# dluvizon/deephar

Measured on NVIDIA H100. Metric: frames/sec (256x256, 16-frame clips, b32), higher is better.
Workload: dtype bf16x3 split (fp32 accumulate, wgmma)

## Files before the change

deephar_b200/csrc/conv_patch.cu:

```cuda
#include "tc_common.cuh"

namespace tcd {
using namespace tc;
using R = tc::Roles<2>;
constexpr int WARP_EPI0 = R::WARP_EPI0, WARP_TMA = R::WARP_TMA, WARP_PATCH = R::WARP_PATCH, NTHREADS = R::NTHREADS,
              REGS_PROD = R::REGS_PROD, REGS_EPI = R::REGS_EPI, REGS_CTRL = R::REGS_CTRL;

constexpr int NWG = 128;
constexpr int NA = 4;
constexpr int NB = 3;
constexpr int MAX_NP = 8;

template <bool LO>
__global__ void __launch_bounds__(NTHREADS, 1)
patch_dense_kernel(const __grid_constant__ PatchParams PP, const __grid_constant__ CUtensorMap map_hi,
                   const __grid_constant__ CUtensorMap map_lo, const __grid_constant__ CUtensorMap map_x) {
    const TcParams& P = PP.t;
    extern __shared__ __align__(1024) uint8_t smem_raw[];
    if (smem_u32(smem_raw) & 1023u) __trap();
    uint8_t* smem = smem_raw;
    const int tid = threadIdx.x;
    const int warp = tid >> 5, lane = tid & 31;
    constexpr bool want_lo = LO;
    const int b_bytes = P.bn_cta * 64;
    uint8_t* b_ring = smem + NA * 2 * A_BYTES;
    uint8_t* patch0 = b_ring + NB * 2 * b_bytes;
    uint64_t* bars = reinterpret_cast<uint64_t*>(patch0 + (size_t)PP.np * PP.patch_stride);
    float* post = reinterpret_cast<float*>(bars + 64);
    constexpr int NB_A = NA + 2 * NA;
    constexpr int NB_P = NB_A + 2 * NB;
    const uint32_t bar_full0 = smem_u32(bars), bar_empty0 = smem_u32(bars + NA), bar_fullb0 = smem_u32(bars + NB_A),
                   bar_emptyb0 = smem_u32(bars + NB_A + NB), bar_pfull0 = smem_u32(bars + NB_P),
                   bar_pempty0 = smem_u32(bars + NB_P + MAX_NP);
    const int n0 = blockIdx.y * P.bn_cta;
    const int nkb = P.n_kblocks;
    const int ntaps = PP.ntaps, ncb = PP.ncb, np = PP.np;

    if (warp == WARP_TMA && lane == 0) {
        tma_prefetch_desc(&map_hi);
        if (want_lo) tma_prefetch_desc(&map_lo);
        tma_prefetch_desc(&map_x);
        for (int s = 0; s < NA; ++s) {
            mbar_init(bar_full0 + 8 * s, (uint32_t)NWG);
            mbar_init(bar_empty0 + 16 * s, 1u);
            mbar_init(bar_empty0 + 16 * s + 8, 1u);
        }
        for (int s = 0; s < NB; ++s) {
            mbar_init(bar_fullb0 + 8 * s, 1);
            mbar_init(bar_emptyb0 + 8 * s, 1);
        }
        for (int s = 0; s < MAX_NP; ++s) {
            mbar_init(bar_pfull0 + 8 * s, 1);
            mbar_init(bar_pempty0 + 8 * s, ntaps == 1 ? (uint32_t)NWG : (uint32_t)(2 * NWG));
        }
        fence_barrier_init();
    }
    __syncthreads();

    const int tiles_mine = ((int)P.n_mtiles - (int)blockIdx.x + (int)gridDim.x - 1) / (int)gridDim.x;
    const int total_g = tiles_mine * nkb;
    const int n_patches = tiles_mine * ncb;
    const int rows_per_tile = BM / PP.tw;

    if (warp < WARP_EPI0) {
        reg_prod<REGS_PROD, R::LAUNCH_REGS>();
        const ConvParams& c = P.c;
        const int w = warp >> 2;
        const int tw = tid & (NWG - 1);
        const int ch4 = tw & 7;
        const int prow = tw >> 3;
        uint32_t poff[8];
        int yy[8], xx[8];
#pragma unroll
        for (int i = 0; i < 8; ++i) {
            const int m = prow + 16 * i;
            const int ty = m / PP.tw, tx = m - ty * PP.tw;
            const int f = ty / PP.ry, r = ty - f * PP.ry;
            poff[i] = (uint32_t)(((f * PP.pr + r * PP.sh) * PP.pc + tx * PP.sw) * (SBK * 4) + ch4 * 16);
            yy[i] = r * PP.sh - PP.pt;
            xx[i] = tx * PP.sw - PP.pl;
        }
        const uint32_t patch_s = smem_u32(patch0);
        const bool relu = c.pre_relu != 0, has_bn = c.pre_scale != nullptr;
        uint32_t aoff[8];
#pragma unroll
        for (int i = 0; i < 8; ++i) aoff[i] = swz64(prow + 16 * i, ch4 * 4);
        int tap = w % ntaps, p = w / ntaps;
        int cb = p % ncb, ti = p / ncb;
        int slot = p % np;
        uint32_t pphase = (uint32_t)(p / np) & 1u;
        int ky = tap / PP.kw, kx = tap - ky * PP.kw;
        int s = w % NA;
        uint32_t it = 0;
        int cb_loaded = -1, ti_masked = -1;
        float4 ps = make_float4(1.f, 1.f, 1.f, 1.f), pb = make_float4(0.f, 0.f, 0.f, 0.f);
        int y0 = 0;
        for (int g = w; g < total_g; g += 2) {
            if (has_bn && cb != cb_loaded) {
                cb_loaded = cb;
                const int ci = cb * SBK + ch4 * 4;
                if (ci < c.Cin) {
                    ps = __ldg(reinterpret_cast<const float4*>(c.pre_scale + ci));
                    pb = __ldg(reinterpret_cast<const float4*>(c.pre_shift + ci));
                } else {
                    ps = make_float4(0.f, 0.f, 0.f, 0.f);
                    pb = make_float4(0.f, 0.f, 0.f, 0.f);
                }
            }
            unsigned okmask = 0xffu;
            if (PP.mask) {
                if (ti != ti_masked) {
                    ti_masked = ti;
                    const int t = blockIdx.x + ti * gridDim.x;
                    y0 = PP.fn > 1 ? 0 : (t * rows_per_tile) % PP.rows_per_frame;
                }
                okmask = 0;
#pragma unroll
                for (int i = 0; i < 8; ++i) {
                    const int iy = y0 * PP.sh + yy[i] + ky, ix = xx[i] + kx;
                    if ((unsigned)iy < (unsigned)PP.vh && (unsigned)ix < (unsigned)PP.vw) okmask |= 1u << i;
                }
            }
            mbar_wait(bar_pfull0 + 8 * slot, pphase);
            const uint32_t base = patch_s + (uint32_t)slot * (uint32_t)PP.patch_stride +
                                  (uint32_t)((ky * PP.pc + kx) * (SBK * 4));
            float4 v[8];
#pragma unroll
            for (int i = 0; i < 8; ++i) v[i] = lds128(base + poff[i]);

            wait_stage_free(bar_empty0, s, it);
            const uint32_t a_hi = smem_u32(smem) + (uint32_t)s * (2 * A_BYTES);
            const uint32_t a_lo = a_hi + A_BYTES;
#pragma unroll
            for (int i = 0; i < 8; ++i) {
                float4 t4 = v[i];
                if (has_bn) {
                    t4.x = fmaf(t4.x, ps.x, pb.x); t4.y = fmaf(t4.y, ps.y, pb.y);
                    t4.z = fmaf(t4.z, ps.z, pb.z); t4.w = fmaf(t4.w, ps.w, pb.w);
                }
                if (relu) {
                    t4.x = fmaxf(t4.x, 0.f); t4.y = fmaxf(t4.y, 0.f); t4.z = fmaxf(t4.z, 0.f); t4.w = fmaxf(t4.w, 0.f);
                }
                if (!((okmask >> i) & 1u)) t4 = make_float4(0.f, 0.f, 0.f, 0.f);
                uint32_t h0, l0, h1, l1;
                split2(t4.x, t4.y, h0, l0);
                split2(t4.z, t4.w, h1, l1);
                asm volatile("st.shared.v2.b32 [%0], {%1, %2};" ::"r"(a_hi + aoff[i]), "r"(h0), "r"(h1) : "memory");
                if (want_lo) asm volatile("st.shared.v2.b32 [%0], {%1, %2};" ::"r"(a_lo + aoff[i]), "r"(l0), "r"(l1) : "memory");
            }
            const bool last_of_patch = tap + 2 >= ntaps;
            if (last_of_patch) mbar_arrive(bar_pempty0 + 8 * slot);
            fence_proxy_async();
            mbar_arrive(bar_full0 + 8 * s);
            s += 2;
            if (s >= NA) { s -= NA; ++it; }
            tap += 2;
            kx += 2;
            while (tap >= ntaps) {
                tap -= ntaps;
                ++p;
                if (++cb == ncb) { cb = 0; ++ti; }
                if (++slot == np) { slot = 0; pphase ^= 1u; }
                ky = 0; kx = tap;
                if (kx >= PP.kw) { kx -= PP.kw; ky = 1; }
            }
            while (kx >= PP.kw) { kx -= PP.kw; ++ky; }
        }
    } else if (warp < WARP_TMA) {
        reg_inc<REGS_EPI>();
        stage_post<R::NEPI>(P, n0, post, tid - 32 * WARP_EPI0);
        const int wg = (warp - WARP_EPI0) >> 2, wt = tid - 32 * WARP_EPI0 - 128 * wg;
        pp_consumer<false, LO, NA, NB>(P, wg, wt, n0, tiles_mine, make_desc64(smem_u32(smem)), make_desc64(smem_u32(b_ring)),
                                       bar_full0, bar_empty0, bar_fullb0, bar_emptyb0, 0u, post, 0);
    } else {
        reg_dec<REGS_CTRL>();
        if (warp == WARP_TMA) {
            if (lane == 0) {
                const uint32_t tx = (uint32_t)(want_lo ? 2 : 1) * (uint32_t)b_bytes;
                for (int g = 0; g < total_g; ++g) {
                    const int p = g / ntaps, tap = g - p * ntaps;
                    const int cb = p % ncb;
                    const int kc = tap * P.c.Cin + cb * SBK;
                    const int sb = g % NB;
                    const uint32_t itb = (uint32_t)(g / NB);
                    if (itb >= 1) mbar_wait_relaxed(bar_emptyb0 + 8 * sb, (itb - 1) & 1, 0u);
                    const uint32_t full = bar_fullb0 + 8 * sb;
                    mbar_arrive_expect_tx(full, tx);
                    const uint32_t b_hi = smem_u32(b_ring + (size_t)sb * (2 * b_bytes));
                    const uint32_t b_lo = b_hi + (uint32_t)b_bytes;
                    tma_load_2d(b_hi, &map_hi, kc, n0, full);
                    if (want_lo) tma_load_2d(b_lo, &map_lo, kc, n0, full);
                }
            }
        } else if (warp == WARP_PATCH) {
            if (lane == 0) {
                for (int p = 0; p < n_patches; ++p) {
                    const int ti = p / ncb, cb = p - ti * ncb;
                    const int t = blockIdx.x + ti * gridDim.x;
                    const int grow = t * rows_per_tile;
                    const int nf = grow / PP.rows_per_frame;
                    const int y0 = grow - nf * PP.rows_per_frame;
                    const int slot = p % np;
                    const uint32_t u = (uint32_t)(p / np);
                    mbar_wait_relaxed(bar_pempty0 + 8 * slot, (u & 1u) ^ 1u, 0u);
                    const uint32_t pf = bar_pfull0 + 8 * slot;
                    mbar_arrive_expect_tx(pf, (uint32_t)PP.patch_bytes);
                    tma_load_4d(smem_u32(patch0 + (size_t)slot * PP.patch_stride), &map_x, cb * SBK, -PP.pl,
                                y0 * PP.sh - PP.pt, nf, pf);
                }
            }
        }
    }
}

static bool plan_geom(const ConvParams& p, PatchParams* g) {
    if (p.sh != 1 || p.sw != 1) return false;
    if (p.kh == 1 && p.kw == 1) {
        const int64_t hw = (int64_t)p.H * p.W;
        int vw = 128;
        while (vw > 1 && (hw % vw) != 0) vw >>= 1;
        if (vw < 8) return false;
        g->tw = vw; g->ry = tc::BM / vw; g->fn = 1; g->pc = vw; g->pr = g->ry;
        g->vw = vw; g->vh = (int)(((int64_t)p.N * hw) / vw);
        g->rows_per_frame = g->vh; g->pt = g->pl = 0; g->kw = 1; g->ntaps = 1;
        return true;
    }
    if (p.Ho != p.H || p.Wo != p.W) return false;
    if (!(p.W == 128 || p.W == 64 || p.W == 32 || p.W == 16 || p.W == 8)) return false;
    const int tr = tc::BM / p.W;
    if (tr <= p.H ? (p.H % tr) != 0 : (tr % p.H) != 0) return false;
    g->tw = p.W;
    g->ry = tr <= p.H ? tr : p.H;
    g->fn = tr <= p.H ? 1 : tr / p.H;
    g->pc = p.W + p.kw - 1;
    g->pr = g->ry + p.kh - 1;
    g->rows_per_frame = p.H; g->vh = p.H; g->vw = p.W;
    g->pt = p.pt; g->pl = p.pl; g->kw = p.kw; g->ntaps = p.kh * p.kw;
    return true;
}

}

bool dh_plan_patch(const dh_ctx* ctx, const ConvParams& p, const dh_packed_w* packed, int precision, tc::PatchPlan* pl) {
    using namespace tc;
    using namespace tcd;
    if (!ctx->dense_patch || !packed->lo) return false;
    if (p.M < 1) return false;
    if ((p.Cin & 7) || (p.ldx & 3) || (reinterpret_cast<uintptr_t>(p.x) & 15) || !bn_pro_aligned(p)) return false;
    if (!packed_fits(packed, p.kh * p.kw * p.Cin, p.Cout)) return false;
    PatchParams& PP = pl->k;
    if (!plan_geom(p, &PP)) return false;
    if (PP.pc > 256 || PP.pr > 256 || PP.fn > 256) return false;
    if ((int64_t)PP.vh * PP.vw * p.ldx * 4 >= (1ll << 40)) return false;
    TcParams& P = PP.t;
    P.c = p;
    P.c.K = p.kh * p.kw * p.Cin;
    P.k_pad = packed->k;
    PP.ncb = (p.Cin + SBK - 1) / SBK;
    P.n_kblocks = PP.ncb * PP.ntaps;
    int gy;
    tile_n(p.Cout, &P.bn_cta, &gy);
    P.precision = (precision == 1) ? 1 : 3;
    P.ks = 0;
    P.n_mtiles = (p.M + BM - 1) / BM;
    P.stages = 2;
    P.dbg = 0;
    PP.sh = 1; PP.sw = 1;
    PP.mask = (p.pre_scale != nullptr && PP.ntaps > 1) ? 1 : 0;
    PP.patch_bytes = SBK * 4 * PP.pc * PP.pr * PP.fn;
    PP.patch_stride = (PP.patch_bytes + 1023) / 1024 * 1024;
    const size_t fixed = (size_t)NA * 2 * A_BYTES + (size_t)NB * 2 * P.bn_cta * 64 + 512 + POST_SMEM;
    const int np = (int)((SMEM_LIMIT - fixed) / (size_t)PP.patch_stride);
    if (np < 2) return false;
    PP.np = np > MAX_NP ? MAX_NP : np;
    pl->w = packed;
    pl->gy = gy;
    pl->smem = fixed + (size_t)PP.np * PP.patch_stride;
    pl->cluster = false;
    return true;
}

int dh_launch_patch(const dh_ctx* ctx, const tc::PatchPlan& pl, cudaStream_t s) {
    using namespace tc;
    using namespace tcd;
    const PatchParams& PP = pl.k;
    const ConvParams& c = PP.t.c;
    const dh_packed_w* w = pl.w;
    const int vn = PP.ntaps == 1 ? 1 : c.N;
    CUtensorMap map_hi, map_lo, map_x;
    if (!make_map_w(&map_hi, w->hi, w->k, w->cout_pad, SBK, PP.t.bn_cta) ||
        !make_map_w(&map_lo, w->lo, w->k, w->cout_pad, SBK, PP.t.bn_cta) ||
        !make_map_x(&map_x, c.x, c.ldx, c.Cin, PP.vw, PP.vh, vn, PP.pc, PP.pr, PP.fn)) {
        dh_set_error("dh_launch_patch: cuTensorMapEncodeTiled failed");
        return -1;
    }
    return pick<true, false>(PP.t.precision == 3, [&](auto lo) {
        return launch_persistent<patch_dense_kernel<lo()>>("dh_launch_patch", ctx, pl, PP.t.n_mtiles, NTHREADS, s,
                                                           map_hi, map_lo, map_x);
    });
}
```

deephar_b200/csrc/tc_common.cuh:

```cuda
#pragma once
#include <cuda.h>
#include <cuda_bf16.h>
#include <type_traits>
#include "common.cuh"
#include "conv_params.cuh"

namespace tc {


constexpr int BM = 128;
constexpr int BK = 64;
constexpr int NPROD = 256;
constexpr int MAX_BN_CTA = 96;
constexpr int ACC_N = MAX_BN_CTA / 2;
constexpr int MH = BM / 64;
constexpr int BM64 = 64;
constexpr int MAX_BN_CTA64 = 144;
constexpr int bn_max(int bm) { return bm == BM64 ? MAX_BN_CTA64 : MAX_BN_CTA; }
template <int Q, int NPW = 2>
struct Roles {
    static constexpr int EPQ = Q;
    static constexpr int NEPI = 128 * Q;
    static constexpr int WARP_EPI0 = 4 * NPW;
    static constexpr int WARP_TMA = WARP_EPI0 + 4 * Q, WARP_PATCH = WARP_TMA + 2;
    static constexpr int NTHREADS = 32 * (WARP_TMA + 4);
    static constexpr int REGS_PROD = Q == 1 ? 168 : (NPW == 1 ? 192 : 88);
    static constexpr int REGS_EPI = Q == 2 && NPW == 2 ? 136 : 144, REGS_CTRL = 32;
    static constexpr int LAUNCH_REGS = NTHREADS <= 512 ? 128 : 96;
    static_assert(128 * NPW * REGS_PROD + NEPI * REGS_EPI + 128 * REGS_CTRL <= NTHREADS * LAUNCH_REGS,
                  "setmaxnreg budget exceeds the CTA's register allocation: the last setmaxnreg.inc would never return");
};
constexpr int A_TILE_BYTES = BM * 128;
constexpr int MAX_STAGES = 4;

struct TcParams {
    ConvParams c;
    int n_kblocks;
    int bn_cta;
    int stages;
    int precision;
    int ks;
    int k_pad;
    int n_mtiles;
    int dbg;
};

struct SepParams {
    TcParams t;
    int patch_stride;
    int patch_bytes;
    int ry, fn;
    int bm;
    int epi_smem;
    int dbg;
};

struct PatchParams {
    TcParams t;
    int np, patch_stride, patch_bytes;
    int ntaps, ncb;
    int tw;
    int ry, fn;
    int pc, pr;
    int rows_per_frame;
    int kw;
    int pt, pl, sh, sw;
    int vh, vw;
    int mask;
};

__device__ __forceinline__ void mbar_wait_relaxed(uint32_t bar, uint32_t parity, uint32_t ns) {
    uint32_t ok;
    for (;;) {
        asm volatile(
            "{\n .reg .pred p;\n mbarrier.try_wait.parity.shared::cta.b64 p, [%1], %2;\n selp.u32 %0, 1, 0, p;\n}"
            : "=r"(ok)
            : "r"(bar), "r"(parity)
            : "memory");
        if (ok) break;
        if (ns) __nanosleep(ns);
    }
}
__device__ __forceinline__ void fence_proxy_async() { asm volatile("fence.proxy.async.shared::cta;" ::: "memory"); }

__device__ __forceinline__ void tma_load_2d(uint32_t dst, const CUtensorMap* map, int c0, int c1, uint32_t bar) {
    asm volatile(
        "cp.async.bulk.tensor.2d.shared::cluster.global.mbarrier::complete_tx::bytes [%0], [%1, {%2, %3}], [%4];"
        ::"r"(dst), "l"(map), "r"(c0), "r"(c1), "r"(bar)
        : "memory");
}
__device__ __forceinline__ void tma_prefetch_desc(const CUtensorMap* map) {
    asm volatile("prefetch.tensormap [%0];" ::"l"(map) : "memory");
}
__device__ __forceinline__ void tma_store_2d(const CUtensorMap* map, uint32_t src, int c0, int c1) {
    asm volatile("cp.async.bulk.tensor.2d.global.shared::cta.bulk_group [%0, {%2, %3}], [%1];"
                 ::"l"(map), "r"(src), "r"(c0), "r"(c1)
                 : "memory");
}
__device__ __forceinline__ void bulk_commit() { asm volatile("cp.async.bulk.commit_group;" ::: "memory"); }
__device__ __forceinline__ void bulk_wait_read() { asm volatile("cp.async.bulk.wait_group.read 0;" ::: "memory"); }
__device__ __forceinline__ void bulk_s2peer(uint32_t dst_cluster, uint32_t src_cta, uint32_t bytes, uint32_t bar_cluster) {
    asm volatile("cp.async.bulk.shared::cluster.shared::cta.mbarrier::complete_tx::bytes [%0], [%1], %2, [%3];"
                 ::"r"(dst_cluster), "r"(src_cta), "r"(bytes), "r"(bar_cluster)
                 : "memory");
}
template <int R> __device__ __forceinline__ void reg_inc() { asm volatile("setmaxnreg.inc.sync.aligned.u32 %0;" ::"n"(R)); }
template <int R> __device__ __forceinline__ void reg_dec() { asm volatile("setmaxnreg.dec.sync.aligned.u32 %0;" ::"n"(R)); }
template <int R, int LAUNCH> __device__ __forceinline__ void reg_prod() {
    if constexpr (R > LAUNCH) reg_inc<R>();
    else if constexpr (R < LAUNCH) reg_dec<R>();
}
__device__ __forceinline__ void mbar_arrive_cluster(uint32_t bar_cluster) {
    asm volatile("mbarrier.arrive.release.cluster.shared::cluster.b64 _, [%0];" ::"r"(bar_cluster) : "memory");
}

__device__ __forceinline__ void wgmma_fence() { asm volatile("wgmma.fence.sync.aligned;" ::: "memory"); }
__device__ __forceinline__ void wgmma_commit() { asm volatile("wgmma.commit_group.sync.aligned;" ::: "memory"); }
template <int N> __device__ __forceinline__ void wgmma_wait() { asm volatile("wgmma.wait_group.sync.aligned %0;" ::"n"(N) : "memory"); }
__device__ __forceinline__ void acc_fence(float& r) { asm volatile("" : "+f"(r)::"memory"); }
template <int N> __device__ __forceinline__ void wgmma_bf16(float* d, uint64_t a, uint64_t b, uint32_t acc);
template <> __device__ __forceinline__ void wgmma_bf16<16>(float* d, uint64_t a, uint64_t b, uint32_t acc) {
    asm volatile(
        "{\n .reg .pred p;\n setp.ne.b32 p, %10, 0;\n"
        " wgmma.mma_async.sync.aligned.m64n16k16.f32.bf16.bf16 {%0, %1, %2, %3, %4, %5, %6, %7}, %8, %9, p, 1, 1, 0, 0;\n}"
        : "+f"(d[0]), "+f"(d[1]), "+f"(d[2]), "+f"(d[3]), "+f"(d[4]), "+f"(d[5]), "+f"(d[6]), "+f"(d[7])
        : "l"(a), "l"(b), "r"(acc));
}
template <> __device__ __forceinline__ void wgmma_bf16<32>(float* d, uint64_t a, uint64_t b, uint32_t acc) {
    asm volatile(
        "{\n .reg .pred p;\n setp.ne.b32 p, %18, 0;\n"
        " wgmma.mma_async.sync.aligned.m64n32k16.f32.bf16.bf16 {%0, %1, %2, %3, %4, %5, %6, %7, %8, %9, %10, %11, %12, %13, %14, %15}, %16, %17, p, 1, 1, 0, 0;\n}"
        : "+f"(d[0]), "+f"(d[1]), "+f"(d[2]), "+f"(d[3]), "+f"(d[4]), "+f"(d[5]), "+f"(d[6]), "+f"(d[7]), "+f"(d[8]), "+f"(d[9]), "+f"(d[10]), "+f"(d[11]), "+f"(d[12]), "+f"(d[13]), "+f"(d[14]), "+f"(d[15])
        : "l"(a), "l"(b), "r"(acc));
}
template <> __device__ __forceinline__ void wgmma_bf16<48>(float* d, uint64_t a, uint64_t b, uint32_t acc) {
    asm volatile(
        "{\n .reg .pred p;\n setp.ne.b32 p, %26, 0;\n"
        " wgmma.mma_async.sync.aligned.m64n48k16.f32.bf16.bf16 {%0, %1, %2, %3, %4, %5, %6, %7, %8, %9, %10, %11, %12, %13, %14, %15, %16, %17, %18, %19, %20, %21, %22, %23}, %24, %25, p, 1, 1, 0, 0;\n}"
        : "+f"(d[0]), "+f"(d[1]), "+f"(d[2]), "+f"(d[3]), "+f"(d[4]), "+f"(d[5]), "+f"(d[6]), "+f"(d[7]), "+f"(d[8]), "+f"(d[9]), "+f"(d[10]), "+f"(d[11]), "+f"(d[12]), "+f"(d[13]), "+f"(d[14]), "+f"(d[15]), "+f"(d[16]), "+f"(d[17]), "+f"(d[18]), "+f"(d[19]), "+f"(d[20]), "+f"(d[21]), "+f"(d[22]), "+f"(d[23])
        : "l"(a), "l"(b), "r"(acc));
}
template <> __device__ __forceinline__ void wgmma_bf16<64>(float* d, uint64_t a, uint64_t b, uint32_t acc) {
    asm volatile(
        "{\n .reg .pred p;\n setp.ne.b32 p, %34, 0;\n"
        " wgmma.mma_async.sync.aligned.m64n64k16.f32.bf16.bf16 {%0, %1, %2, %3, %4, %5, %6, %7, %8, %9, %10, %11, %12, %13, %14, %15, %16, %17, %18, %19, %20, %21, %22, %23, %24, %25, %26, %27, %28, %29, %30, %31}, %32, %33, p, 1, 1, 0, 0;\n}"
        : "+f"(d[0]), "+f"(d[1]), "+f"(d[2]), "+f"(d[3]), "+f"(d[4]), "+f"(d[5]), "+f"(d[6]), "+f"(d[7]), "+f"(d[8]), "+f"(d[9]), "+f"(d[10]), "+f"(d[11]), "+f"(d[12]), "+f"(d[13]), "+f"(d[14]), "+f"(d[15]), "+f"(d[16]), "+f"(d[17]), "+f"(d[18]), "+f"(d[19]), "+f"(d[20]), "+f"(d[21]), "+f"(d[22]), "+f"(d[23]), "+f"(d[24]), "+f"(d[25]), "+f"(d[26]), "+f"(d[27]), "+f"(d[28]), "+f"(d[29]), "+f"(d[30]), "+f"(d[31])
        : "l"(a), "l"(b), "r"(acc));
}
template <> __device__ __forceinline__ void wgmma_bf16<80>(float* d, uint64_t a, uint64_t b, uint32_t acc) {
    asm volatile(
        "{\n .reg .pred p;\n setp.ne.b32 p, %42, 0;\n"
        " wgmma.mma_async.sync.aligned.m64n80k16.f32.bf16.bf16 {%0, %1, %2, %3, %4, %5, %6, %7, %8, %9, %10, %11, %12, %13, %14, %15, %16, %17, %18, %19, %20, %21, %22, %23, %24, %25, %26, %27, %28, %29, %30, %31, %32, %33, %34, %35, %36, %37, %38, %39}, %40, %41, p, 1, 1, 0, 0;\n}"
        : "+f"(d[0]), "+f"(d[1]), "+f"(d[2]), "+f"(d[3]), "+f"(d[4]), "+f"(d[5]), "+f"(d[6]), "+f"(d[7]), "+f"(d[8]), "+f"(d[9]), "+f"(d[10]), "+f"(d[11]), "+f"(d[12]), "+f"(d[13]), "+f"(d[14]), "+f"(d[15]), "+f"(d[16]), "+f"(d[17]), "+f"(d[18]), "+f"(d[19]), "+f"(d[20]), "+f"(d[21]), "+f"(d[22]), "+f"(d[23]), "+f"(d[24]), "+f"(d[25]), "+f"(d[26]), "+f"(d[27]), "+f"(d[28]), "+f"(d[29]), "+f"(d[30]), "+f"(d[31]), "+f"(d[32]), "+f"(d[33]), "+f"(d[34]), "+f"(d[35]), "+f"(d[36]), "+f"(d[37]), "+f"(d[38]), "+f"(d[39])
        : "l"(a), "l"(b), "r"(acc));
}
template <> __device__ __forceinline__ void wgmma_bf16<96>(float* d, uint64_t a, uint64_t b, uint32_t acc) {
    asm volatile(
        "{\n .reg .pred p;\n setp.ne.b32 p, %50, 0;\n"
        " wgmma.mma_async.sync.aligned.m64n96k16.f32.bf16.bf16 {%0, %1, %2, %3, %4, %5, %6, %7, %8, %9, %10, %11, %12, %13, %14, %15, %16, %17, %18, %19, %20, %21, %22, %23, %24, %25, %26, %27, %28, %29, %30, %31, %32, %33, %34, %35, %36, %37, %38, %39, %40, %41, %42, %43, %44, %45, %46, %47}, %48, %49, p, 1, 1, 0, 0;\n}"
        : "+f"(d[0]), "+f"(d[1]), "+f"(d[2]), "+f"(d[3]), "+f"(d[4]), "+f"(d[5]), "+f"(d[6]), "+f"(d[7]), "+f"(d[8]), "+f"(d[9]), "+f"(d[10]), "+f"(d[11]), "+f"(d[12]), "+f"(d[13]), "+f"(d[14]), "+f"(d[15]), "+f"(d[16]), "+f"(d[17]), "+f"(d[18]), "+f"(d[19]), "+f"(d[20]), "+f"(d[21]), "+f"(d[22]), "+f"(d[23]), "+f"(d[24]), "+f"(d[25]), "+f"(d[26]), "+f"(d[27]), "+f"(d[28]), "+f"(d[29]), "+f"(d[30]), "+f"(d[31]), "+f"(d[32]), "+f"(d[33]), "+f"(d[34]), "+f"(d[35]), "+f"(d[36]), "+f"(d[37]), "+f"(d[38]), "+f"(d[39]), "+f"(d[40]), "+f"(d[41]), "+f"(d[42]), "+f"(d[43]), "+f"(d[44]), "+f"(d[45]), "+f"(d[46]), "+f"(d[47])
        : "l"(a), "l"(b), "r"(acc));
}

template <> __device__ __forceinline__ void wgmma_bf16<144>(float* d, uint64_t a, uint64_t b, uint32_t acc) {
    asm volatile(
        "{\n .reg .pred p;\n setp.ne.b32 p, %74, 0;\n"
        " wgmma.mma_async.sync.aligned.m64n144k16.f32.bf16.bf16 {%0, %1, %2, %3, %4, %5, %6, %7, %8, %9, %10, %11, %12, %13, %14, %15, %16, %17, %18, %19, %20, %21, %22, %23, %24, %25, %26, %27, %28, %29, %30, %31, %32, %33, %34, %35, %36, %37, %38, %39, %40, %41, %42, %43, %44, %45, %46, %47, %48, %49, %50, %51, %52, %53, %54, %55, %56, %57, %58, %59, %60, %61, %62, %63, %64, %65, %66, %67, %68, %69, %70, %71}, %72, %73, p, 1, 1, 0, 0;\n}"
        : "+f"(d[0]), "+f"(d[1]), "+f"(d[2]), "+f"(d[3]), "+f"(d[4]), "+f"(d[5]), "+f"(d[6]), "+f"(d[7]), "+f"(d[8]), "+f"(d[9]), "+f"(d[10]), "+f"(d[11]), "+f"(d[12]), "+f"(d[13]), "+f"(d[14]), "+f"(d[15]), "+f"(d[16]), "+f"(d[17]), "+f"(d[18]), "+f"(d[19]), "+f"(d[20]), "+f"(d[21]), "+f"(d[22]), "+f"(d[23]), "+f"(d[24]), "+f"(d[25]), "+f"(d[26]), "+f"(d[27]), "+f"(d[28]), "+f"(d[29]), "+f"(d[30]), "+f"(d[31]), "+f"(d[32]), "+f"(d[33]), "+f"(d[34]), "+f"(d[35]), "+f"(d[36]), "+f"(d[37]), "+f"(d[38]), "+f"(d[39]), "+f"(d[40]), "+f"(d[41]), "+f"(d[42]), "+f"(d[43]), "+f"(d[44]), "+f"(d[45]), "+f"(d[46]), "+f"(d[47]), "+f"(d[48]), "+f"(d[49]), "+f"(d[50]), "+f"(d[51]), "+f"(d[52]), "+f"(d[53]), "+f"(d[54]), "+f"(d[55]), "+f"(d[56]), "+f"(d[57]), "+f"(d[58]), "+f"(d[59]), "+f"(d[60]), "+f"(d[61]), "+f"(d[62]), "+f"(d[63]), "+f"(d[64]), "+f"(d[65]), "+f"(d[66]), "+f"(d[67]), "+f"(d[68]), "+f"(d[69]), "+f"(d[70]), "+f"(d[71])
        : "l"(a), "l"(b), "r"(acc));
}

__device__ __forceinline__ uint64_t make_desc(uint32_t smem_addr) {
    return (uint64_t)((smem_addr >> 4) & 0x3FFF) | (1ull << 16) | ((uint64_t)(1024 >> 4) << 32) | (1ull << 62);
}


__device__ __forceinline__ void split2(float a, float b, uint32_t& hi, uint32_t& lo) {
    __nv_bfloat162 h = __floats2bfloat162_rn(a, b);
    float ra = a - __low2float(h), rb = b - __high2float(h);
    __nv_bfloat162 l = __floats2bfloat162_rn(ra, rb);
    hi = *reinterpret_cast<uint32_t*>(&h);
    lo = *reinterpret_cast<uint32_t*>(&l);
}

__device__ __forceinline__ uint32_t swz(int row, int k) {
    return (uint32_t)(row * 128 + ((((k >> 3) ^ (row & 7)) << 4) | ((k & 7) << 1)));
}


constexpr int SBK = 32;
constexpr int A_BYTES = BM * 64;
__device__ __forceinline__ void tma_load_4d(uint32_t dst, const CUtensorMap* map, int c0, int c1, int c2, int c3,
                                            uint32_t bar) {
    asm volatile(
        "cp.async.bulk.tensor.4d.shared::cluster.global.mbarrier::complete_tx::bytes [%0], [%1, {%2, %3, %4, %5}], [%6];"
        ::"r"(dst), "l"(map), "r"(c0), "r"(c1), "r"(c2), "r"(c3), "r"(bar)
        : "memory");
}

__device__ __forceinline__ void tma_prefetch_4d(const CUtensorMap* map, int c0, int c1, int c2, int c3) {
    asm volatile("cp.async.bulk.prefetch.tensor.4d.L2.global [%0, {%1, %2, %3, %4}];"
                 ::"l"(map), "r"(c0), "r"(c1), "r"(c2), "r"(c3) : "memory");
}

__device__ __forceinline__ uint64_t make_desc64(uint32_t smem_addr) {
    return (uint64_t)((smem_addr >> 4) & 0x3FFF) | (1ull << 16) | ((uint64_t)(512 >> 4) << 32) | (2ull << 62);
}
__device__ __forceinline__ uint32_t swz64(int row, int k) {
    return (uint32_t)(row * 64 + ((((k >> 3) ^ ((row >> 1) & 3)) << 4) | ((k & 7) << 1)));
}

__device__ __forceinline__ float4 lds128(uint32_t a) {
    float4 v;
    asm volatile("ld.shared.v4.f32 {%0, %1, %2, %3}, [%4];" : "=f"(v.x), "=f"(v.y), "=f"(v.z), "=f"(v.w) : "r"(a) : "memory");
    return v;
}

__device__ __forceinline__ void wait_stage_free(uint32_t bar_empty0, int s, uint32_t it, uint32_t ns = 0) {
    if (it >= 1) mbar_wait_relaxed(bar_empty0 + 16 * s + 8 * ((it - 1) & 1), ((it - 1) >> 1) & 1, ns);
}


template <int N, int MHT, int ACCN>
__device__ __forceinline__ void acc_fence_all(float (&acc)[MHT][ACCN]) {
#pragma unroll
    for (int h = 0; h < MHT; ++h)
#pragma unroll
        for (int i = 0; i < N / 2; ++i) acc_fence(acc[h][i]);
}

template <int N, int NK16, bool LO, int MHT, int ACCN>
__device__ __forceinline__ void wg_issue_kblock(float (&acc)[MHT][ACCN], uint64_t da, uint32_t a_half16, uint32_t alo16,
                                                uint64_t db, uint32_t blo16, bool first) {
    wgmma_fence();
#pragma unroll
    for (int k = 0; k < NK16; ++k) {
        const uint32_t acc0 = (first && k == 0) ? 0u : 1u;
#pragma unroll
        for (int h = 0; h < MHT; ++h) {
            const uint64_t a = da + (uint64_t)(h * a_half16 + 2 * k);
            wgmma_bf16<N>(acc[h], a, db + 2 * k, acc0);
            if (LO) {
                wgmma_bf16<N>(acc[h], a + alo16, db + 2 * k, 1u);
                wgmma_bf16<N>(acc[h], a, db + blo16 + 2 * k, 1u);
            }
        }
    }
    wgmma_commit();
}

template <int N, int NK16, bool LO, int MHT, int ACCN, class Stage, class Release>
__device__ __forceinline__ void wg_tile_n(float (&acc)[MHT][ACCN], int nkb, uint32_t a_half16, uint32_t alo16,
                                          uint32_t blo16, bool mma, Stage& stage, Release& release) {
    for (int kb = 0; kb < nkb; ++kb) {
        uint64_t da, db;
        stage(kb, da, db);
        if (mma) {
            acc_fence_all<N>(acc);
            wg_issue_kblock<N, NK16, LO>(acc, da, a_half16, alo16, db, blo16, kb == 0);
        }
        wgmma_wait<1>();
        acc_fence_all<N>(acc);
        if (kb > 0) release(kb - 1);
    }
    wgmma_wait<0>();
    acc_fence_all<N>(acc);
    release(nkb - 1);
}

template <int NK16, bool LO, int MHT, int ACCN, class Stage, class Release>
__device__ __forceinline__ void wg_tile(int bn, float (&acc)[MHT][ACCN], int nkb, uint32_t a_half16, uint32_t alo16,
                                        uint32_t blo16, bool mma, Stage&& stage, Release&& release) {
    if constexpr (ACCN == MAX_BN_CTA64 / 2) {
        wg_tile_n<MAX_BN_CTA64, NK16, LO>(acc, nkb, a_half16, alo16, blo16, mma, stage, release);
    } else {
        switch (bn) {
        case 16: wg_tile_n<16, NK16, LO>(acc, nkb, a_half16, alo16, blo16, mma, stage, release); break;
        case 32: wg_tile_n<32, NK16, LO>(acc, nkb, a_half16, alo16, blo16, mma, stage, release); break;
        case 48: wg_tile_n<48, NK16, LO>(acc, nkb, a_half16, alo16, blo16, mma, stage, release); break;
        case 64: wg_tile_n<64, NK16, LO>(acc, nkb, a_half16, alo16, blo16, mma, stage, release); break;
        case 80: wg_tile_n<80, NK16, LO>(acc, nkb, a_half16, alo16, blo16, mma, stage, release); break;
        default: wg_tile_n<96, NK16, LO>(acc, nkb, a_half16, alo16, blo16, mma, stage, release); break;
        }
    }
}

__device__ __forceinline__ void pp_pass(int wg) { asm volatile("bar.arrive %0, 256;" ::"r"(6 + wg) : "memory"); }
__device__ __forceinline__ void pp_wait(int wg) { asm volatile("bar.sync %0, 256;" ::"r"(7 - wg) : "memory"); }

__device__ __forceinline__ void wg_release(uint32_t bar, int wg, int wt, bool remote, uint32_t peer) {
    asm volatile("bar.sync %0, 128;" ::"r"(4 + wg) : "memory");
    if (wt == 0) {
        mbar_arrive(bar);
        if (remote) mbar_arrive_cluster(mapa_peer(bar, peer));
    }
}

__device__ __forceinline__ float2 ldg2(const float* p) { return __ldg(reinterpret_cast<const float2*>(p)); }

constexpr int post_smem(int bm) { return 2 * bn_max(bm) * 4; }
constexpr int POST_SMEM = post_smem(BM);
template <int NEPI, int BNMAX = MAX_BN_CTA>
__device__ __forceinline__ void stage_post(const TcParams& P, int n0, float* post, int ct) {
    const ConvParams& c = P.c;
    if (c.post_scale) {
        for (int j = ct; j < P.bn_cta; j += NEPI) {
            const int co = n0 + j;
            post[j] = co < c.Cout ? __ldg(c.post_scale + co) : 0.f;
            post[BNMAX + j] = co < c.Cout ? __ldg(c.post_shift + co) : 0.f;
        }
    }
    asm volatile("bar.sync 2, %0;" ::"n"(NEPI) : "memory");
}

__device__ __forceinline__ void prefetch_l2(const float* p) { asm volatile("prefetch.global.L2 [%0];" ::"l"(p)); }
template <int TBM = BM>
__device__ __forceinline__ void wg_prefetch_res(const TcParams& P, int m0, int n0, int wt) {
    const ConvParams& c = P.c;
#ifdef DH_ABLATE
    if (P.dbg & 32) return;
#endif
    const int m = m0 + wt;
    if (wt >= TBM || m >= c.M) return;
    const int last = min(P.bn_cta, c.Cout - n0) - 1;
    if (c.res0) {
        const float* r = c.res0 + (size_t)m * c.ldr0 + n0;
        for (int k = 0; k < last; k += 32) prefetch_l2(r + k);
        prefetch_l2(r + last);
    }
    if (c.res1) {
        const float* r = c.res1 + res1_src(c, m) * c.ldr1 + n0;
        for (int k = 0; k < last; k += 32) prefetch_l2(r + k);
        prefetch_l2(r + last);
    }
}

template <int MHT, int ACCN>
__device__ __forceinline__ void wg_epilogue(const TcParams& P, const float (&acc)[MHT][ACCN], int m0, int n0, int wt,
                                            const float* post) {
    const ConvParams& c = P.c;
#ifdef DH_ABLATE
    if (P.dbg & 32) return;
#endif
    const int rq = 16 * (wt >> 5) + ((wt & 31) >> 2);
    const int c0 = n0 + 2 * (wt & 3);
    const bool v2 = !((c.ldo | c.Cout) & 1) && !(reinterpret_cast<uintptr_t>(c.out) & 7) &&
                    (!c.res0 || (!(c.ldr0 & 1) && !(reinterpret_cast<uintptr_t>(c.res0) & 7))) &&
                    (!c.res1 || (!(c.ldr1 & 1) && !(reinterpret_cast<uintptr_t>(c.res1) & 7)));
    const bool relu = c.post_relu != 0, has_post = c.post_scale != nullptr;
    const int ncol = min(P.bn_cta - 2 * (wt & 3), c.Cout - c0);
    const float* sc = post + (c0 - n0);
    const float* sh = sc + 2 * ACCN;
    constexpr int JC = 3;
    static_assert((ACCN / 4) % JC == 0, "column groups per batch");
#pragma unroll
    for (int h = 0; h < MHT; ++h)
#pragma unroll
        for (int hr = 0; hr < 2; ++hr) {
            const int m = m0 + 64 * h + rq + 8 * hr;
            if (m >= c.M) continue;
            float* orow = c.out + (size_t)m * c.ldo + c0;
            const float* r0row = c.res0 ? c.res0 + (size_t)m * c.ldr0 + c0 : nullptr;
            const float* r1row = c.res1 ? c.res1 + res1_src(c, m) * c.ldr1 + c0 : nullptr;
            if (v2) {
#pragma unroll
                for (int j0 = 0; j0 < ACCN / 4; j0 += JC) {
                    if (8 * j0 >= P.bn_cta) break;
                    float2 ra[JC], rb[JC];
#pragma unroll
                    for (int jj = 0; jj < JC; ++jj) {
                        if (8 * (j0 + jj) < ncol) {
                            if (r0row) ra[jj] = ldg2(r0row + 8 * (j0 + jj));
                            if (r1row) rb[jj] = ldg2(r1row + 8 * (j0 + jj));
                        }
                    }
#pragma unroll
                    for (int jj = 0; jj < JC; ++jj) {
                        const int j = j0 + jj;
                        if (8 * j < ncol) {
                            float2 v = make_float2(acc[h][4 * j + 2 * hr], acc[h][4 * j + 2 * hr + 1]);
                            if (has_post)
                                v = ffma2(v, *reinterpret_cast<const float2*>(sc + 8 * j),
                                          *reinterpret_cast<const float2*>(sh + 8 * j));
                            if (relu) v = make_float2(fmaxf(v.x, 0.f), fmaxf(v.y, 0.f));
                            if (r0row) v = fadd2(v, ra[jj]);
                            if (r1row) v = fadd2(v, rb[jj]);
                            *reinterpret_cast<float2*>(orow + 8 * j) = v;
                        }
                    }
                }
                continue;
            }
#pragma unroll
            for (int j = 0; j < ACCN / 4; ++j) {
                if (8 * j >= P.bn_cta) break;
#pragma unroll
                for (int e = 0; e < 2; ++e) {
                    const int k = 8 * j + e;
                    if (k < ncol) {
                        float t = acc[h][4 * j + 2 * hr + e];
                        if (has_post) t = fmaf(t, sc[k], sh[k]);
                        if (relu) t = fmaxf(t, 0.f);
                        if (r0row) t += __ldg(r0row + k);
                        if (r1row) t += __ldg(r1row + k);
                        orow[k] = t;
                    }
                }
            }
        }
}

struct EpiSmem {
    float* buf;
    const float* r1;
    uint32_t full0, empty;
    const CUtensorMap* map_out;
};
constexpr int EPI_BUF_BYTES = BM64 * MAX_BN_CTA64 * 4, EPI_R1_BYTES = BM64 / 4 * MAX_BN_CTA64 * 4;

template <int ACCN>
__device__ __forceinline__ void wg_epilogue_smem(const TcParams& P, const float (&acc)[1][ACCN], int ti, int m0, int n0,
                                                 int wg, int wt, const float* post, const EpiSmem& es) {
    static_assert(2 * ACCN == MAX_BN_CTA64, "the buffer holds one 64 x 144 tile");
    const ConvParams& c = P.c;
    mbar_wait(es.full0 + 8 * wg, (uint32_t)(ti >> 1) & 1);
#ifdef DH_ABLATE
    const bool skip = P.dbg & 32;
#else
    constexpr bool skip = false;
#endif
    if (!skip) {
        const int rq = 16 * (wt >> 5) + ((wt & 31) >> 2);
        const int cq = 2 * (wt & 3);
        const bool relu = c.post_relu != 0, has_post = c.post_scale != nullptr, r0 = c.res0 != nullptr;
        const float* sc = post + cq;
        const float* sh = sc + 2 * ACCN;
#pragma unroll
        for (int hr = 0; hr < 2; ++hr) {
            const int r = rq + 8 * hr;
            float* row = es.buf + r * MAX_BN_CTA64 + cq;
            const float* r1row = es.r1 ? es.r1 + (res1_src(c, m0 + r) - (size_t)(m0 / 4)) * MAX_BN_CTA64 + cq : nullptr;
#pragma unroll
            for (int j = 0; j < ACCN / 4; ++j) {
                float2 v = make_float2(acc[0][4 * j + 2 * hr], acc[0][4 * j + 2 * hr + 1]);
                if (has_post)
                    v = ffma2(v, *reinterpret_cast<const float2*>(sc + 8 * j), *reinterpret_cast<const float2*>(sh + 8 * j));
                if (relu) v = make_float2(fmaxf(v.x, 0.f), fmaxf(v.y, 0.f));
                if (r0) v = fadd2(v, *reinterpret_cast<const float2*>(row + 8 * j));
                if (r1row) v = fadd2(v, *reinterpret_cast<const float2*>(r1row + 8 * j));
                *reinterpret_cast<float2*>(row + 8 * j) = v;
            }
        }
        fence_proxy_async();
    }
    asm volatile("bar.sync %0, 128;" ::"r"(4 + wg) : "memory");
    if (wt == 0) {
        if (!skip) {
            tma_store_2d(es.map_out, smem_u32(es.buf), n0, m0);
            bulk_commit();
            bulk_wait_read();
        }
        mbar_arrive(es.empty);
    }
}

template <bool SHARE, bool LO, int NA, int NB, int TBM = BM>
__device__ __forceinline__ void pp_consumer(const TcParams& P, int wg, int wt, int n0, int tiles_mine, uint64_t dbase,
                                            uint64_t dbase_b, uint32_t bar_full0, uint32_t bar_empty0,
                                            uint32_t bar_fullb0, uint32_t bar_emptyb0, uint32_t rank, const float* post,
                                            int dbg, EpiSmem es = {}) {
    static_assert(NA % 2 == 0 || !SHARE, "each A stage has one producing CTA of the pair");
    const int nkb = P.n_kblocks;
    const int b_bytes = P.bn_cta * 64;
    constexpr int a_bytes = TBM * 64;
    float acc[TBM / 64][bn_max(TBM) / 2];
    const uint32_t sta16 = (2 * a_bytes) >> 4, stb16 = (uint32_t)(2 * b_bytes) >> 4, alo16 = a_bytes >> 4,
                   blo16 = (uint32_t)b_bytes >> 4, half16 = (64 * 64) >> 4;
    for (int ti = wg; ti < tiles_mine; ti += 2) {
        const int g0 = ti * nkb, m0 = ((int)blockIdx.x + ti * (int)gridDim.x) * TBM;
        if (ti > 0) pp_wait(wg);
        if (!es.buf) wg_prefetch_res<TBM>(P, m0, n0, wt);
        wg_tile<SBK / 16, LO>(
            P.bn_cta, acc, nkb, half16, alo16, blo16, !(dbg & 64),
            [&](int kb, uint64_t& da, uint64_t& db) {
                const int g = g0 + kb, s = g % NA, sb = g % NB;
                if (!(dbg & 128)) mbar_wait(bar_full0 + 8 * s, (uint32_t)(g / NA) & 1);
                mbar_wait(bar_fullb0 + 8 * sb, (uint32_t)(g / NB) & 1);
                if (kb == nkb - 1 && ti + 1 < tiles_mine) pp_pass(wg);
                da = dbase + (uint64_t)((uint32_t)s * sta16);
                db = dbase_b + (uint64_t)((uint32_t)sb * stb16);
            },
            [&](int kb) {
                const int g = g0 + kb, s = g % NA;
                const uint32_t producer = (uint32_t)(s & 1);
                wg_release(bar_empty0 + 16 * s + 8 * ((g / NA) & 1), wg, wt, SHARE && producer != rank, producer);
                if (wt == 0) mbar_arrive(bar_emptyb0 + 8 * (g % NB));
            });
        if constexpr (TBM == BM64) {
            if (es.buf) {
                wg_epilogue_smem(P, acc, ti, m0, n0, wg, wt, post, es);
                continue;
            }
        }
        wg_epilogue(P, acc, m0, n0, wt, post);
    }
}

typedef CUresult (*EncodeTiledFn)(CUtensorMap*, CUtensorMapDataType, cuuint32_t, void*, const cuuint64_t*,
                                  const cuuint64_t*, const cuuint32_t*, const cuuint32_t*, CUtensorMapInterleave,
                                  CUtensorMapSwizzle, CUtensorMapL2promotion, CUtensorMapFloatOOBfill);

static inline EncodeTiledFn get_encode() {
    static EncodeTiledFn fn = nullptr;
    if (!fn) {
        void* p = nullptr;
        cudaDriverEntryPointQueryResult qres;
        if (cudaGetDriverEntryPoint("cuTensorMapEncodeTiled", &p, cudaEnableDefault, &qres) == cudaSuccess &&
            qres == cudaDriverEntryPointSuccess)
            fn = (EncodeTiledFn)p;
    }
    return fn;
}

static inline bool make_map_w(CUtensorMap* map, const void* base, int k_pad, int rows, int kblk, int box_rows) {
    EncodeTiledFn enc = get_encode();
    if (!enc) return false;
    cuuint64_t dims[2] = {(cuuint64_t)k_pad, (cuuint64_t)rows};
    cuuint64_t strides[1] = {(cuuint64_t)k_pad * 2};
    cuuint32_t box[2] = {(cuuint32_t)kblk, (cuuint32_t)box_rows};
    cuuint32_t estr[2] = {1, 1};
    return enc(map, CU_TENSOR_MAP_DATA_TYPE_BFLOAT16, 2, const_cast<void*>(base), dims, strides, box, estr,
               CU_TENSOR_MAP_INTERLEAVE_NONE, kblk == BK ? CU_TENSOR_MAP_SWIZZLE_128B : CU_TENSOR_MAP_SWIZZLE_64B,
               CU_TENSOR_MAP_L2_PROMOTION_L2_256B, CU_TENSOR_MAP_FLOAT_OOB_FILL_NONE) == CUDA_SUCCESS;
}

static inline bool make_map_x(CUtensorMap* map, const float* x, int ldx, int c, int w, int h, int n, int pc, int pr,
                              int fn) {
    EncodeTiledFn enc = get_encode();
    if (!enc) return false;
    cuuint64_t dims[4] = {(cuuint64_t)c, (cuuint64_t)w, (cuuint64_t)h, (cuuint64_t)n};
    cuuint64_t strides[3] = {(cuuint64_t)ldx * 4, (cuuint64_t)w * ldx * 4, (cuuint64_t)h * w * ldx * 4};
    cuuint32_t box[4] = {(cuuint32_t)SBK, (cuuint32_t)pc, (cuuint32_t)pr, (cuuint32_t)fn};
    cuuint32_t estr[4] = {1, 1, 1, 1};
    return enc(map, CU_TENSOR_MAP_DATA_TYPE_FLOAT32, 4, const_cast<float*>(x), dims, strides, box, estr,
               CU_TENSOR_MAP_INTERLEAVE_NONE, CU_TENSOR_MAP_SWIZZLE_NONE, CU_TENSOR_MAP_L2_PROMOTION_L2_256B,
               CU_TENSOR_MAP_FLOAT_OOB_FILL_NONE) == CUDA_SUCCESS;
}

static inline bool make_map_rows(CUtensorMap* map, const float* p, int cols, int rows, int ld, int box_cols, int box_rows) {
    EncodeTiledFn enc = get_encode();
    if (!enc) return false;
    cuuint64_t dims[2] = {(cuuint64_t)cols, (cuuint64_t)rows};
    cuuint64_t strides[1] = {(cuuint64_t)ld * 4};
    cuuint32_t box[2] = {(cuuint32_t)box_cols, (cuuint32_t)box_rows};
    cuuint32_t estr[2] = {1, 1};
    return enc(map, CU_TENSOR_MAP_DATA_TYPE_FLOAT32, 2, const_cast<float*>(p), dims, strides, box, estr,
               CU_TENSOR_MAP_INTERLEAVE_NONE, CU_TENSOR_MAP_SWIZZLE_NONE, CU_TENSOR_MAP_L2_PROMOTION_L2_256B,
               CU_TENSOR_MAP_FLOAT_OOB_FILL_NONE) == CUDA_SUCCESS;
}
static inline bool tma_view_ok(const float* p, int ld) { return !(reinterpret_cast<uintptr_t>(p) & 15) && !(ld & 3); }

static inline void tile_n(int cout, int* bn_cta, int* gy, int max_bn = MAX_BN_CTA) {
    const int cp = (cout + 15) / 16 * 16;
    const int g = (cp + max_bn - 1) / max_bn;
    *bn_cta = ((cp + g - 1) / g + 15) / 16 * 16;
    *gy = g;
}

constexpr size_t SMEM_LIMIT = 227 * 1024;

static inline bool packed_fits(const dh_packed_w* w, int K, int cout) {
    return w->k == dh_tc_k_pad(K) && w->cout_pad == dh_tc_cout_pad(cout);
}

static inline bool bn_pro_aligned(const ConvParams& p) {
    return !p.pre_scale || !((reinterpret_cast<uintptr_t>(p.pre_scale) | reinterpret_cast<uintptr_t>(p.pre_shift)) & 15);
}

static inline bool tc_layer_ok(const ConvParams& p, const dh_packed_w* w, int K) {
    return p.M >= 1 && packed_fits(w, K, p.Cout) && (int64_t)p.N * p.H * p.W * p.ldx < (1ll << 31);
}

static inline bool sep_layer_ok(const ConvParams& p, const dh_packed_w* w) {
    if (!tc_layer_ok(p, w, p.Cin) || (reinterpret_cast<uintptr_t>(p.x) & 15) || !bn_pro_aligned(p)) return false;
    if (!(p.kh == p.kw && (p.kh == 3 || p.kh == 5))) return false;
    if (p.sh != 1 || p.sw != 1) return false;
    if (p.Ho != p.H || p.Wo != p.W) return false;
    if (p.W < 4 || (BM % p.W) != 0 || (p.W & 3) || (p.H & 3)) return false;
    if ((p.Cin & 1) || (p.ldx & 1)) return false;
    if ((reinterpret_cast<uintptr_t>(p.w_dw) & 7) != 0) return false;
    return p.M % (4 * p.W) == 0;
}

template <class Params>
struct Plan {
    Params k;
    const dh_packed_w* w;
    int gy;
    size_t smem;
    bool cluster;
};
using TcPlan = Plan<TcParams>;
using SepPlan = Plan<SepParams>;
using PatchPlan = Plan<PatchParams>;

template <auto V, auto... Vs, class T, class F>
static inline auto pick(T v, F&& f) {
    if constexpr (sizeof...(Vs) == 0) return f(std::integral_constant<decltype(V), V>{});
    else return v == V ? f(std::integral_constant<decltype(V), V>{}) : pick<Vs...>(v, f);
}

static inline int persistent_gx(const dh_ctx* ctx, int gy, int n_mtiles) {
    int gx = ctx->num_sms / gy;
    if (gx < 1) gx = 1;
    if (gx > n_mtiles) gx = n_mtiles;
    return gx;
}

template <auto Kernel, class Params, class... Maps>
static inline int launch_persistent(const char* who, const dh_ctx* ctx, const Plan<Params>& pl, int n_mtiles,
                                    int nthreads, cudaStream_t s, const Maps&... maps) {
    cudaError_t e = ensure_smem<Kernel>(pl.smem);
    if (e == cudaSuccess) {
        cudaLaunchConfig_t cfg = {};
        cfg.gridDim = dim3(persistent_gx(ctx, pl.gy, n_mtiles), pl.gy);
        cfg.blockDim = dim3(nthreads);
        cfg.dynamicSmemBytes = pl.smem;
        cfg.stream = s;
        cudaLaunchAttribute at[1];
        if (pl.cluster) {
            at[0].id = cudaLaunchAttributeClusterDimension;
            at[0].val.clusterDim.x = 1; at[0].val.clusterDim.y = 2; at[0].val.clusterDim.z = 1;
            cfg.attrs = at;
            cfg.numAttrs = 1;
        }
        e = cudaLaunchKernelEx(&cfg, Kernel, pl.k, maps...);
    }
    if (e != cudaSuccess) {
        dh_set_error("%s: launch setup failed: %s", who, cudaGetErrorString(e));
        return (int)e;
    }
    return 0;
}

}

bool dh_plan_patch(const dh_ctx* ctx, const ConvParams& p, const dh_packed_w* packed, int precision, tc::PatchPlan* pl);
int dh_launch_patch(const dh_ctx* ctx, const tc::PatchPlan& pl, cudaStream_t s);
bool dh_plan_sep_tma(const dh_ctx* ctx, const ConvParams& p, const dh_packed_w* packed, int precision, tc::SepPlan* pl);
int dh_launch_sep_tma(const dh_ctx* ctx, const tc::SepPlan& pl, cudaStream_t s);
bool dh_plan_conv_tc(const dh_ctx* ctx, const ConvParams& p, const dh_packed_w* packed, bool separable, int precision,
                     tc::TcPlan* pl);
int dh_launch_conv_tc(const dh_ctx* ctx, const tc::TcPlan& pl, cudaStream_t s);
```

Before: 4100.

## Route stride-2 convolutions through patch kernel using TMA element strides per tap

Extends the patch-based implicit-GEMM conv kernel to handle stride-2 kxk convolutions without pre-BN. Each kernel tap becomes its own sub-patch, loaded by a TMA descriptor with element stride 2, so the patch in shared memory is already decimated and the producers read it densely. Previously these convs fell back to a different path. The cost is one TMA patch load per tap instead of one shared halo patch, plus an extra template variant and stricter shape constraints on Wo and Ho.

```diff
diff --git a/deephar_b200/csrc/conv_patch.cu b/deephar_b200/csrc/conv_patch.cu
--- a/deephar_b200/csrc/conv_patch.cu
+++ b/deephar_b200/csrc/conv_patch.cu
@@ -11,7 +11,7 @@
 constexpr int NB = 3;
 constexpr int MAX_NP = 8;
 
-template <bool LO>
+template <bool LO, bool SUB>
 __global__ void __launch_bounds__(NTHREADS, 1)
 patch_dense_kernel(const __grid_constant__ PatchParams PP, const __grid_constant__ CUtensorMap map_hi,
                    const __grid_constant__ CUtensorMap map_lo, const __grid_constant__ CUtensorMap map_x) {
@@ -34,7 +34,7 @@
                    bar_pempty0 = smem_u32(bars + NB_P + MAX_NP);
     const int n0 = blockIdx.y * P.bn_cta;
     const int nkb = P.n_kblocks;
-    const int ntaps = PP.ntaps, ncb = PP.ncb, np = PP.np;
+    const int ntaps = PP.ntaps, ncb = PP.ncb, nsub = SUB ? PP.nsub : 1, np = PP.np;
 
     if (warp == WARP_TMA && lane == 0) {
         tma_prefetch_desc(&map_hi);
@@ -59,7 +59,7 @@
 
     const int tiles_mine = ((int)P.n_mtiles - (int)blockIdx.x + (int)gridDim.x - 1) / (int)gridDim.x;
     const int total_g = tiles_mine * nkb;
-    const int n_patches = tiles_mine * ncb;
+    const int n_patches = tiles_mine * ncb * nsub;
     const int rows_per_tile = BM / PP.tw;
 
     if (warp < WARP_EPI0) {
@@ -76,7 +76,7 @@
             const int m = prow + 16 * i;
             const int ty = m / PP.tw, tx = m - ty * PP.tw;
             const int f = ty / PP.ry, r = ty - f * PP.ry;
-            poff[i] = (uint32_t)(((f * PP.pr + r * PP.sh) * PP.pc + tx * PP.sw) * (SBK * 4) + ch4 * 16);
+            poff[i] = (uint32_t)(((f * PP.pr + r) * PP.pc + tx) * (SBK * 4) + ch4 * 16);
             yy[i] = r * PP.sh - PP.pt;
             xx[i] = tx * PP.sw - PP.pl;
         }
@@ -86,7 +86,7 @@
 #pragma unroll
         for (int i = 0; i < 8; ++i) aoff[i] = swz64(prow + 16 * i, ch4 * 4);
         int tap = w % ntaps, p = w / ntaps;
-        int cb = p % ncb, ti = p / ncb;
+        int cb = p % ncb, sub = (p / ncb) % nsub, ti = p / (ncb * nsub);
         int slot = p % np;
         uint32_t pphase = (uint32_t)(p / np) & 1u;
         int ky = tap / PP.kw, kx = tap - ky * PP.kw;
@@ -159,7 +159,10 @@
             while (tap >= ntaps) {
                 tap -= ntaps;
                 ++p;
-                if (++cb == ncb) { cb = 0; ++ti; }
+                if (++cb == ncb) {
+                    cb = 0;
+                    if (++sub == nsub) { sub = 0; ++ti; }
+                }
                 if (++slot == np) { slot = 0; pphase ^= 1u; }
                 ky = 0; kx = tap;
                 if (kx >= PP.kw) { kx -= PP.kw; ky = 1; }
@@ -179,8 +182,9 @@
                 const uint32_t tx = (uint32_t)(want_lo ? 2 : 1) * (uint32_t)b_bytes;
                 for (int g = 0; g < total_g; ++g) {
                     const int p = g / ntaps, tap = g - p * ntaps;
-                    const int cb = p % ncb;
-                    const int kc = tap * P.c.Cin + cb * SBK;
+                    const int q = p / ncb, cb = p - q * ncb;
+                    const int kt = SUB ? q % nsub : tap;
+                    const int kc = kt * P.c.Cin + cb * SBK;
                     const int sb = g % NB;
                     const uint32_t itb = (uint32_t)(g / NB);
                     if (itb >= 1) mbar_wait_relaxed(bar_emptyb0 + 8 * sb, (itb - 1) & 1, 0u);
@@ -195,7 +199,9 @@
         } else if (warp == WARP_PATCH) {
             if (lane == 0) {
                 for (int p = 0; p < n_patches; ++p) {
-                    const int ti = p / ncb, cb = p - ti * ncb;
+                    const int q = p / ncb, cb = p - q * ncb;
+                    const int ti = q / nsub, sub = q - ti * nsub;
+                    const int ky = sub / PP.kw, kx = sub - ky * PP.kw;
                     const int t = blockIdx.x + ti * gridDim.x;
                     const int grow = t * rows_per_tile;
                     const int nf = grow / PP.rows_per_frame;
@@ -205,8 +211,8 @@
                     mbar_wait_relaxed(bar_pempty0 + 8 * slot, (u & 1u) ^ 1u, 0u);
                     const uint32_t pf = bar_pfull0 + 8 * slot;
                     mbar_arrive_expect_tx(pf, (uint32_t)PP.patch_bytes);
-                    tma_load_4d(smem_u32(patch0 + (size_t)slot * PP.patch_stride), &map_x, cb * SBK, -PP.pl,
-                                y0 * PP.sh - PP.pt, nf, pf);
+                    tma_load_4d(smem_u32(patch0 + (size_t)slot * PP.patch_stride), &map_x, cb * SBK, kx - PP.pl,
+                                y0 * PP.sh - PP.pt + ky, nf, pf);
                 }
             }
         }
@@ -214,6 +220,21 @@
 }
 
 static bool plan_geom(const ConvParams& p, PatchParams* g) {
+    g->nsub = 1; g->sh = p.sh; g->sw = p.sw;
+    if (p.sh == 2 && p.sw == 2 && p.kh > 1 && p.kw > 1) {
+        if (p.pre_scale) return false;
+        if (!(p.Wo == 128 || p.Wo == 64 || p.Wo == 32 || p.Wo == 16 || p.Wo == 8)) return false;
+        const int tr = tc::BM / p.Wo;
+        if (tr <= p.Ho ? (p.Ho % tr) != 0 : (tr % p.Ho) != 0) return false;
+        g->tw = p.Wo;
+        g->ry = tr <= p.Ho ? tr : p.Ho;
+        g->fn = tr <= p.Ho ? 1 : tr / p.Ho;
+        g->pc = p.Wo;
+        g->pr = g->ry;
+        g->rows_per_frame = p.Ho; g->vh = p.H; g->vw = p.W;
+        g->pt = p.pt; g->pl = p.pl; g->kw = p.kw; g->ntaps = 1; g->nsub = p.kh * p.kw;
+        return true;
+    }
     if (p.sh != 1 || p.sw != 1) return false;
     if (p.kh == 1 && p.kw == 1) {
         const int64_t hw = (int64_t)p.H * p.W;
@@ -250,14 +271,14 @@
     if (!packed_fits(packed, p.kh * p.kw * p.Cin, p.Cout)) return false;
     PatchParams& PP = pl->k;
     if (!plan_geom(p, &PP)) return false;
-    if (PP.pc > 256 || PP.pr > 256 || PP.fn > 256) return false;
+    if (PP.pc * PP.sw > 256 || PP.pr * PP.sh > 256 || PP.fn > 256) return false;
     if ((int64_t)PP.vh * PP.vw * p.ldx * 4 >= (1ll << 40)) return false;
     TcParams& P = PP.t;
     P.c = p;
     P.c.K = p.kh * p.kw * p.Cin;
     P.k_pad = packed->k;
     PP.ncb = (p.Cin + SBK - 1) / SBK;
-    P.n_kblocks = PP.ncb * PP.ntaps;
+    P.n_kblocks = PP.ncb * PP.nsub * PP.ntaps;
     int gy;
     tile_n(p.Cout, &P.bn_cta, &gy);
     P.precision = (precision == 1) ? 1 : 3;
@@ -265,7 +286,6 @@
     P.n_mtiles = (p.M + BM - 1) / BM;
     P.stages = 2;
     P.dbg = 0;
-    PP.sh = 1; PP.sw = 1;
     PP.mask = (p.pre_scale != nullptr && PP.ntaps > 1) ? 1 : 0;
     PP.patch_bytes = SBK * 4 * PP.pc * PP.pr * PP.fn;
     PP.patch_stride = (PP.patch_bytes + 1023) / 1024 * 1024;
@@ -286,16 +306,18 @@
     const PatchParams& PP = pl.k;
     const ConvParams& c = PP.t.c;
     const dh_packed_w* w = pl.w;
-    const int vn = PP.ntaps == 1 ? 1 : c.N;
+    const int vn = c.kh * c.kw == 1 ? 1 : c.N;
     CUtensorMap map_hi, map_lo, map_x;
     if (!make_map_w(&map_hi, w->hi, w->k, w->cout_pad, SBK, PP.t.bn_cta) ||
         !make_map_w(&map_lo, w->lo, w->k, w->cout_pad, SBK, PP.t.bn_cta) ||
-        !make_map_x(&map_x, c.x, c.ldx, c.Cin, PP.vw, PP.vh, vn, PP.pc, PP.pr, PP.fn)) {
+        !make_map_x(&map_x, c.x, c.ldx, c.Cin, PP.vw, PP.vh, vn, PP.pc, PP.pr, PP.fn, PP.sw)) {
         dh_set_error("dh_launch_patch: cuTensorMapEncodeTiled failed");
         return -1;
     }
     return pick<true, false>(PP.t.precision == 3, [&](auto lo) {
-        return launch_persistent<patch_dense_kernel<lo()>>("dh_launch_patch", ctx, pl, PP.t.n_mtiles, NTHREADS, s,
-                                                           map_hi, map_lo, map_x);
+        return pick<true, false>(PP.nsub > 1, [&](auto sub) {
+            return launch_persistent<patch_dense_kernel<lo(), sub()>>("dh_launch_patch", ctx, pl, PP.t.n_mtiles,
+                                                                      NTHREADS, s, map_hi, map_lo, map_x);
+        });
     });
 }
diff --git a/deephar_b200/csrc/tc_common.cuh b/deephar_b200/csrc/tc_common.cuh
--- a/deephar_b200/csrc/tc_common.cuh
+++ b/deephar_b200/csrc/tc_common.cuh
@@ -59,6 +59,7 @@
     TcParams t;
     int np, patch_stride, patch_bytes;
     int ntaps, ncb;
+    int nsub;
     int tw;
     int ry, fn;
     int pc, pr;
@@ -535,13 +536,13 @@
 }
 
 static inline bool make_map_x(CUtensorMap* map, const float* x, int ldx, int c, int w, int h, int n, int pc, int pr,
-                              int fn) {
+                              int fn, int es = 1) {
     EncodeTiledFn enc = get_encode();
     if (!enc) return false;
     cuuint64_t dims[4] = {(cuuint64_t)c, (cuuint64_t)w, (cuuint64_t)h, (cuuint64_t)n};
     cuuint64_t strides[3] = {(cuuint64_t)ldx * 4, (cuuint64_t)w * ldx * 4, (cuuint64_t)h * w * ldx * 4};
-    cuuint32_t box[4] = {(cuuint32_t)SBK, (cuuint32_t)pc, (cuuint32_t)pr, (cuuint32_t)fn};
-    cuuint32_t estr[4] = {1, 1, 1, 1};
+    cuuint32_t box[4] = {(cuuint32_t)SBK, (cuuint32_t)(pc * es), (cuuint32_t)(pr * es), (cuuint32_t)fn};
+    cuuint32_t estr[4] = {1, (cuuint32_t)es, (cuuint32_t)es, 1};
     return enc(map, CU_TENSOR_MAP_DATA_TYPE_FLOAT32, 4, const_cast<float*>(x), dims, strides, box, estr,
                CU_TENSOR_MAP_INTERLEAVE_NONE, CU_TENSOR_MAP_SWIZZLE_NONE, CU_TENSOR_MAP_L2_PROMOTION_L2_256B,
                CU_TENSOR_MAP_FLOAT_OOB_FILL_NONE) == CUDA_SUCCESS;
```

Measured after the change: 4162 (median of 6 runs). +1.5%, better.
